# wejpurvis/DIS_project

Hardware: AMD Instinct MI355X
Metric: log-marginal-likelihood evals/sec + fp64 Cholesky GFLOP/s at N=16384 (higher is better)
Workload: dtype f64; 1 GPU; configs[1]: one MLL eval per rank, 64 genes x 256 timepoints, N=16384, fp64; N=16384, genes=64, parallelism=replicas1, exchange=none

## Files before the change

### dis_project_amd/csrc/lfm_chol.hip

```cpp
#include <cstdint>

#include "lfm_chol.h"
#include "lfm_chol_dev.h"

namespace lfm {

static constexpr int STEP_KS = 16;
constexpr int PANEL_TIMEOUT = STATUS_TIMEOUT;
__device__ __forceinline__ void timeout_at(int* status, int why) {
  atomicMin(status, PANEL_TIMEOUT);
  atomicCAS(status + 1, 0, why);
}

template <int SRC>
__device__ __forceinline__ double row_bcast_t(double v) {
  const long long b = __double_as_longlong(v);
  const int lo = __builtin_amdgcn_mov_dpp((int)b, 0x150 + SRC, 0xf, 0xf, false);
  const int hi = __builtin_amdgcn_mov_dpp((int)(b >> 32), 0x150 + SRC, 0xf, 0xf, false);
  return __longlong_as_double(((long long)hi << 32) | (unsigned)lo);
}
__device__ __forceinline__ double row_bcast(double v, int src) {
  switch (src) {
    case 0: return row_bcast_t<0>(v);
    case 1: return row_bcast_t<1>(v);
    case 2: return row_bcast_t<2>(v);
    case 3: return row_bcast_t<3>(v);
    case 4: return row_bcast_t<4>(v);
    case 5: return row_bcast_t<5>(v);
    case 6: return row_bcast_t<6>(v);
    case 7: return row_bcast_t<7>(v);
    case 8: return row_bcast_t<8>(v);
    case 9: return row_bcast_t<9>(v);
    case 10: return row_bcast_t<10>(v);
    case 11: return row_bcast_t<11>(v);
    case 12: return row_bcast_t<12>(v);
    case 13: return row_bcast_t<13>(v);
    case 14: return row_bcast_t<14>(v);
    default: return row_bcast_t<15>(v);
  }
}

template <int SRC>
__device__ __forceinline__ double row_bcast64_t(double v) {
  return __builtin_amdgcn_mov_dpp(v, 0x150 + SRC, 0xf, 0xf, false);
}
__device__ __forceinline__ double row_bcast64(double v, int src) {
  switch (src) {
    case 0: return row_bcast64_t<0>(v);
    case 1: return row_bcast64_t<1>(v);
    case 2: return row_bcast64_t<2>(v);
    case 3: return row_bcast64_t<3>(v);
    case 4: return row_bcast64_t<4>(v);
    case 5: return row_bcast64_t<5>(v);
    case 6: return row_bcast64_t<6>(v);
    case 7: return row_bcast64_t<7>(v);
    case 8: return row_bcast64_t<8>(v);
    case 9: return row_bcast64_t<9>(v);
    case 10: return row_bcast64_t<10>(v);
    case 11: return row_bcast64_t<11>(v);
    case 12: return row_bcast64_t<12>(v);
    case 13: return row_bcast64_t<13>(v);
    case 14: return row_bcast64_t<14>(v);
    default: return row_bcast64_t<15>(v);
  }
}

__device__ __forceinline__ void pin16(double (&p)[16]) {
  asm volatile("" : "+v"(p[0]), "+v"(p[1]), "+v"(p[2]), "+v"(p[3]), "+v"(p[4]), "+v"(p[5]),
               "+v"(p[6]), "+v"(p[7]), "+v"(p[8]), "+v"(p[9]), "+v"(p[10]), "+v"(p[11]),
               "+v"(p[12]), "+v"(p[13]), "+v"(p[14]), "+v"(p[15]));
}

template <bool COH>
__device__ __forceinline__ void st1(double* p, double v) {
  if (COH) __hip_atomic_store(p, v, __ATOMIC_RELAXED, __HIP_MEMORY_SCOPE_AGENT);
  else *p = v;
}
typedef unsigned u32x4v __attribute__((ext_vector_type(4)));
__device__ __forceinline__ void st2_wt(double* base, unsigned off, double a, double b) {
  const __amdgpu_buffer_rsrc_t r = __builtin_amdgcn_make_buffer_rsrc(base, 0, 0x7fffffff, 0x00020000);
  const double2v v = {a, b};
  __builtin_amdgcn_raw_buffer_store_b128(__builtin_bit_cast(u32x4v, v), r, off, 0, 16 );
}
template <bool COH>
__device__ __forceinline__ double ld1(const double* p) {
  if (COH) return __hip_atomic_load(p, __ATOMIC_RELAXED, __HIP_MEMORY_SCOPE_AGENT);
  return *p;
}

__device__ __forceinline__ double rsqrt_nr(double x) {
  double y = __builtin_amdgcn_rsq(x);
  y = y * fma(-0.5 * x * y, y, 1.5);
  y = y * fma(-0.5 * x * y, y, 1.5);
  return y;
}


template <int PH>
__device__ __forceinline__ void potrf_block(double* __restrict__ Mb, double* __restrict__ A,
                                            int64_t lda, int64_t kb, int64_t npiv,
                                            double* __restrict__ dinv,
                                            double* __restrict__ parts, int k,
                                            int* __restrict__ status,
                                            double* __restrict__ Li = nullptr,
                                            unsigned long long* __restrict__ pst = nullptr) {
  auto pstamp = [&](int p) {
    if (pst && threadIdx.x == 0) pst[p] = __builtin_amdgcn_s_memrealtime();
  };
  __shared__ double pvs[NB];
  __shared__ double ipv[NB];
  __shared__ double red[4];
  __shared__ int redi[4];
  int tid = threadIdx.x;
  asm volatile("" : "+v"(tid));
  const int lane = tid & 63, w = tid >> 6;
  const int li = lane & 15, lk = lane >> 4;
#define MS(r, q) Mb[((((r) >> 4) * (((r) >> 4) + 1) / 2) + ((q) >> 4)) * (IB * (IB + 1)) + \
                    ((r) & 15) * (IB + 1) + ((q) & 15)]

  constexpr int LB = (PH & 32) ? 32 : 16;
#pragma unroll
  for (int hb = 0; hb < 32 / LB; ++hb) {
    double2 v[LB];
#pragma unroll
    for (int u = 0; u < LB; ++u) {
      const int idx = tid + 256 * (u + LB * hb), r = idx >> 6, c2 = idx & 63;
      if ((2 * c2) >> 4 <= r >> 4)
        v[u] = (PH & 8) ? ld2<(PH & 16) != 0>(&A[(kb + r) * lda + kb + 2 * c2])
                        : double2{(r == 2 * c2) ? 2.0 : 0.0, (r == 2 * c2 + 1) ? 2.0 : 0.0};
    }
#pragma unroll
    for (int u = 0; u < LB; ++u) {
      const int idx = tid + 256 * (u + LB * hb), r = idx >> 6, c2 = idx & 63;
      if ((2 * c2) >> 4 <= r >> 4) {
        MS(r, 2 * c2) = v[u].x;
        MS(r, 2 * c2 + 1) = v[u].y;
      }
    }
  }
  __syncthreads();

  auto leaf = [&](int cb) {
    const int c0 = cb * IB;
    double d[IB], pv[IB], yv[IB];
#pragma unroll
    for (int q = 0; q < IB; ++q) d[q] = (lane < IB && q <= lane) ? MS(c0 + li, c0 + q) : 0.0;
    if constexpr ((PH & 128) != 0) {
      double dc = row_bcast64(d[0], 0);
      if (kb + c0 >= npiv) dc = 1.0;
      double y = rsqrt_1nr(dc);
#pragma unroll
      for (int c = 0; c < IB; ++c) {
        pv[c] = dc;
        yv[c] = y;
        d[c] = (lane == c) ? dc * y : d[c] * y;
        if (c + 1 < IB) {
          d[c + 1] = fma(-d[c], row_bcast64(d[c], c + 1), d[c + 1]);
          double dn = row_bcast64(d[c + 1], c + 1);
          if (kb + c0 + c + 1 >= npiv) dn = 1.0;
          const double r = __builtin_amdgcn_rsq(dn);
          const double hh = -0.5 * dn;
          const int REM = IB - c - 2, K = (REM + 3) / 4;
          double t1 = 0.0, t2 = 0.0, yn = 0.0;
#pragma unroll
          for (int part = 0; part < 4; ++part) {
            double bq[4];
#pragma unroll
            for (int i = 0; i < 4; ++i) {
              const int q = c + 2 + part * K + i;
              if (i < K && q < IB) bq[i] = row_bcast64(d[c], q);
            }
            __builtin_amdgcn_sched_barrier(0);
#pragma unroll
            for (int i = 0; i < 4; ++i) {
              const int q = c + 2 + part * K + i;
              if (i < K && q < IB) d[q] = fma(-d[c], bq[i], d[q]);
            }
            if (part == 0) t1 = hh * r;
            if (part == 1) t2 = fma(t1, r, 1.5);
            if (part == 2) yn = r * t2;
            __builtin_amdgcn_sched_barrier(0);
          }
          dc = dn;
          y = yn;
        }
      }
    } else {
#pragma unroll
      for (int c = 0; c < IB; ++c) {
        double dc = row_bcast(d[c], c);
        if (kb + c0 + c >= npiv) dc = 1.0;
        const double y = rsqrt_1nr(dc);
        pv[c] = dc;
        yv[c] = y;
        d[c] = (lane == c) ? dc * y : d[c] * y;
#pragma unroll
        for (int q = c + 1; q < IB; ++q) d[q] = fma(-d[c], row_bcast(d[c], q), d[q]);
      }
    }
    if (lane < IB) {
#pragma unroll
      for (int q = 0; q < IB; ++q)
        if (q <= lane) MS(c0 + lane, c0 + q) = d[q];
    }
    double pvl = 0.0, yvl = 0.0;
#pragma unroll
    for (int c = 0; c < IB; ++c) {
      pvl = (lane == c) ? pv[c] : pvl;
      yvl = (lane == c) ? yv[c] : yvl;
    }
    if (lane < IB) {
      pvs[c0 + lane] = pvl;
      ipv[c0 + lane] = yvl;
    }
  };
  auto tile_update = [&](int i0, int j0, int c0) {
    const int bi = __builtin_amdgcn_readfirstlane(i0 >> 4);
    const int bj = __builtin_amdgcn_readfirstlane(j0 >> 4);
    const int bc = __builtin_amdgcn_readfirstlane(c0 >> 4);
    double* C = Mb + (bi * (bi + 1) / 2 + bj) * (IB * (IB + 1));
    const double* Pa = Mb + (bi * (bi + 1) / 2 + bc) * (IB * (IB + 1));
    const double* Pb = Mb + (bj * (bj + 1) / 2 + bc) * (IB * (IB + 1));
    double4v acc;
#pragma unroll
    for (int r = 0; r < 4; ++r) acc[r] = C[(lk + 4 * r) * (IB + 1) + li];
#pragma unroll
    for (int ks = 0; ks < IB / 4; ++ks)
      acc = mfma16(-Pa[li * (IB + 1) + ks * 4 + lk], Pb[li * (IB + 1) + ks * 4 + lk], acc);
#pragma unroll
    for (int r = 0; r < 4; ++r) C[(lk + 4 * r) * (IB + 1) + li] = acc[r];
  };
  auto tri_tile = [](int t, int* ti, int* tj) {
    int r = 0;
    while ((r + 1) * (r + 2) / 2 <= t) ++r;
    *ti = r;
    *tj = t - r * (r + 1) / 2;
  };
#define LI(r, q) Li[((((r) >> 4) * (((r) >> 4) + 1) / 2) + ((q) >> 4)) * (IB * (IB + 1)) + \
                    ((r) & 15) * (IB + 1) + ((q) & 15)]
  auto sweep_pinned = [](double (&p)[IB], const double* Ld, const double* y) {
    double lc[IB], ln[IB], yc = y[0], yn = 0.0;
#pragma unroll
    for (int q = 1; q < IB; ++q) lc[q] = Ld[q * (IB + 1)];
#pragma unroll
    for (int c = 0; c < IB; ++c) {
      if (c + 1 < IB) {
        yn = y[c + 1];
#pragma unroll
        for (int q = c + 2; q < IB; ++q) ln[q] = Ld[q * (IB + 1) + c + 1];
      }
      p[c] = p[c] * yc;
#pragma unroll
      for (int q = c + 1; q < IB; ++q) p[q] = fma(-p[c], lc[q], p[q]);
      pin16(p);
      yc = yn;
#pragma unroll
      for (int q = c + 2; q < IB; ++q) lc[q] = ln[q];
    }
  };
  auto dinv_block = [&](int I) {
    const int c0 = I * IB;
    const int bd = __builtin_amdgcn_readfirstlane(I);
    const double* Ld = Mb + (bd * (bd + 1) / 2 + bd) * (IB * (IB + 1));
    double x[IB];
#pragma unroll
    for (int r = 0; r < IB; ++r) x[r] = (li == r) ? 1.0 : 0.0;
    if constexpr ((PH & 512) != 0) {
      sweep_pinned(x, Ld, ipv + c0);
    } else {
#pragma unroll
      for (int r = 0; r < IB; ++r) {
        x[r] = x[r] * ipv[c0 + r];
#pragma unroll
        for (int q = r + 1; q < IB; ++q) x[q] = fma(-Ld[q * (IB + 1) + r], x[r], x[q]);
      }
    }
    if (lane < IB) {
#pragma unroll
      for (int r = 0; r < IB; ++r) LI(c0 + r, c0 + lane) = x[r];
    }
  };
  auto linv_block = [&](int I, int J) {
    I = __builtin_amdgcn_readfirstlane(I);
    J = __builtin_amdgcn_readfirstlane(J);
    auto blk = [&](int bi, int bj) { return (bi * (bi + 1) / 2 + bj) * (IB * (IB + 1)); };
    double4v sacc = {0, 0, 0, 0};
    for (int K = J; K < I; ++K) {
      const double* a = Mb + blk(I, K);
      const double* b = Li + blk(K, J);
#pragma unroll
      for (int ks = 0; ks < IB / 4; ++ks)
        sacc = mfma16(a[li * (IB + 1) + 4 * ks + lk], b[(4 * ks + lk) * (IB + 1) + li], sacc);
    }
    const double* d = Li + blk(I, I);
    double4v o = {0, 0, 0, 0};
#pragma unroll
    for (int ks = 0; ks < IB / 4; ++ks) o = mfma16(d[li * (IB + 1) + 4 * ks + lk], sacc[ks], o);
    double* out = Li + blk(I, J);
#pragma unroll
    for (int r = 0; r < 4; ++r) out[(lk + 4 * r) * (IB + 1) + li] = -o[r];
  };
  if ((PH & 1) && w == 0) leaf(0);
  __syncthreads();
  pstamp(0);
#pragma unroll 1
  for (int ib = 0; ib < NB / IB; ++ib) {
// ... 624 lines not shown
  double* Xb = g.X + (i0 - g.tr0 + wr + lk) * W + c0 + wc + li;
#pragma unroll
  for (int ir = 0; ir < 8; ++ir)
#pragma unroll
    for (int jr = 0; jr < JR; ++jr) {
      Xb[(ir * 4) * W + jr * 16] = ACC(ir, jr);
      if (i0 + wr + ir * 4 + lk == g.n) g.zvec[g.tk0 + c0 + wc + jr * 16 + li] = ACC(ir, jr);
    }
#undef ACC
  if (st) {
    __syncthreads();
    stamp_max(st + 3);
    add_dur(6);
  }
  return true;
}

template <int TR>
__device__ __forceinline__ void step_body(const StepArgs& g, unsigned long long* ran = nullptr) {
  constexpr int SUB = ST / TR;
  __shared__ double sPbuf[(64 + ST) * (STEP_KS + LDP)];
  double (*sP)[KB + LDP] = reinterpret_cast<double (*)[KB + LDP]>(sPbuf);
  double (*sPu)[STEP_KS + LDP] = reinterpret_cast<double (*)[STEP_KS + LDP]>(sPbuf);
  const int64_t b = blockIdx.x;
  const int cnt[3] = {g.na, g.nr, g.nt};
  const int64_t width[2] = {pad8(g.na), pad8(g.nr)};
  int seg = 0;
  int64_t base = 0;
  while (seg < 2 && b >= base + width[seg]) {
    base += width[seg];
    ++seg;
  }
  int64_t lo, hi;
  tall_or_xcd_range(seg, cnt[seg], b - base, &lo, &hi);
  const int64_t u = lo;
  if (u >= hi) return;
  const int role = seg + 1;
  if (ran && threadIdx.x == 0) *ran = ((unsigned long long)role << 32) | (unsigned long long)u;
  unsigned long long* const st = g.stamps;
  if (st) stamp_max(st, true);
  const unsigned long long t_unit = st ? __builtin_amdgcn_s_memrealtime() : 0;
  auto add_dur = [&](int slot) {
    if (threadIdx.x == 0)
      __hip_atomic_fetch_add(st + slot, __builtin_amdgcn_s_memrealtime() - t_unit,
                             __ATOMIC_RELAXED, __HIP_MEMORY_SCOPE_AGENT);
  };
  if (role == 1) {
    syrk_unit<true, TR, true, STEP_KS>(g.A, g.lda, g.s0, g.px, g.kd, g.T, 0, g.wn, u, g.wn, sPu,
                                       0, g.n, g.pad_end, g.zero_from,
                                       g.gen.tab ? &g.gen : nullptr);
    __builtin_amdgcn_s_waitcnt(0);
    __syncthreads();
    const int trow = g.wn + (int)(u / (SUB * g.wn));
    if (threadIdx.x == 0 && g.a_done)
      __hip_atomic_fetch_add(&g.a_done[trow], 1u, __ATOMIC_RELAXED, __HIP_MEMORY_SCOPE_AGENT);
    if (threadIdx.x == 0 && g.xready && trow < g.wn + g.lead)
      __hip_atomic_fetch_add(g.xready, 1u, __ATOMIC_RELAXED, __HIP_MEMORY_SCOPE_AGENT);
    if (st) {
      stamp_max(st + 1);
      stamp_max(st + 3);
      add_dur(7);
    }
    return;
  }
  if (role == 2) {
    unsigned long long c0 = 0, r0 = 0;
    if (st) {
      c0 = __builtin_amdgcn_s_memtime();
      r0 = __builtin_amdgcn_s_memrealtime();
    }
    const bool lead = syrk_unit<true, TR, false, STEP_KS>(g.A, g.lda, g.s0, g.px, g.kd, g.T,
                                                          g.wn, g.T, u + g.rest_off, 0, sPu,
                                                          g.xready ? g.wn + g.lead : 0, g.n,
                                                          g.pad_end, g.zero_from,
                                                          g.gen.tab ? &g.gen : nullptr);
    if (lead) bump_after_stores(g.xready);
    if (st) {
      __syncthreads();
      stamp_max(st + 1);
      stamp_max(st + 3);
      if (threadIdx.x == 0) {
        __hip_atomic_fetch_add(st + 4, __builtin_amdgcn_s_memtime() - c0, __ATOMIC_RELAXED,
                               __HIP_MEMORY_SCOPE_AGENT);
        __hip_atomic_fetch_add(st + 5, __builtin_amdgcn_s_memrealtime() - r0, __ATOMIC_RELAXED,
                               __HIP_MEMORY_SCOPE_AGENT);
      }
    }
    return;
  }
  tall_unit(g, u, sP, st, t_unit);
}

template <int TR>
__device__ __forceinline__ void step_traced(const StepArgs& g) {
  __shared__ unsigned long long t0;
  __shared__ unsigned long long ran;
  if (threadIdx.x == 0) {
    t0 = __builtin_amdgcn_s_memrealtime();
    ran = 0;
  }
  __syncthreads();
  step_body<TR>(g, &ran);
  __syncthreads();
  if (threadIdx.x == 0) {
    const int64_t b = blockIdx.x;
    unsigned hw, xcc;
    asm volatile("s_getreg_b32 %0, hwreg(HW_REG_HW_ID)" : "=s"(hw));
    asm volatile("s_getreg_b32 %0, hwreg(HW_REG_XCC_ID)" : "=s"(xcc));
    unsigned long long* r = g.trace + 4 * b;
    r[0] = t0;
    r[1] = __builtin_amdgcn_s_memrealtime();
    r[2] = (unsigned long long)hw | ((unsigned long long)xcc << 32);
    r[3] = (g.trace_tag << 40) | ran;
  }
}

__global__ __launch_bounds__(256, 4) void step_kernel(StepArgs g) { step_body<64>(g); }
__global__ __launch_bounds__(256, 4) void helper_update_kernel(StepArgs g) { step_body<64>(g); }
__global__ __launch_bounds__(256, 4) void step_kernel_traced(StepArgs g) { step_traced<64>(g); }
__global__ __launch_bounds__(256, 4) void helper_update_kernel_traced(StepArgs g) {
  step_traced<64>(g);
}

static_assert(MB_DOUBLES >= 64 * (NB + 1) && MB_DOUBLES >= (64 + ST) * (KB + LDP), "LDS union");

__device__ __forceinline__ bool wait_counter(unsigned* p, unsigned target, unsigned limit,
                                             const int* status) {
  __shared__ int ok;
  if (threadIdx.x == 0) ok = spin_until<true>(p, target, limit, status);
  __syncthreads();
  __builtin_amdgcn_fence(__ATOMIC_ACQUIRE, "agent");
  return ok;
}

__global__ __launch_bounds__(256) void panel_kernel(double* __restrict__ A, int64_t lda,
                                                    int64_t kb, int64_t pkb, int pkd,
                                                    int64_t npiv, double* __restrict__ dinv,
                                                    double* __restrict__ parts, int k,
                                                    int* __restrict__ status,
                                                    unsigned* __restrict__ sync, unsigned epoch,
                                                    unsigned spin) {
  extern __shared__ __attribute__((aligned(16))) double smem[];
  __builtin_amdgcn_s_setprio(3);
  const int tid = threadIdx.x, lane = tid & 63, w = tid >> 6;
  const int wr = (w >> 1) * 32, wc = (w & 1) * 64;
  const int li = lane & 15, lk = lane >> 4;
  const int b = blockIdx.x;
  const int64_t i0 = b < 2 ? kb + 64 * b : kb + NB + 64 * (int64_t)(b - 2);
  double* Cb = A + (i0 + wr + lk) * lda + kb + wc + li;
  const int ld4 = (int)(4 * lda);
  double acc[8][4];
#pragma unroll
  for (int ir = 0; ir < 8; ++ir)
#pragma unroll
    for (int jr = 0; jr < 4; ++jr) acc[ir][jr] = -Cb[ir * ld4 + jr * 16];
  if (pkd > 0)
    gemm_accumulate<64>(A + i0 * lda + pkb, lda, A + kb * lda + pkb, lda, pkd, acc,
                        reinterpret_cast<double (*)[KB + LDP]>(smem));
  if (b < 2) {
#pragma unroll
    for (int ir = 0; ir < 8; ++ir)
#pragma unroll
      for (int jr = 0; jr < 4; ++jr) Cb[ir * ld4 + jr * 16] = -acc[ir][jr];
    __threadfence();
    __syncthreads();
    if (tid == 0) __hip_atomic_fetch_add(&sync[1], 1u, __ATOMIC_RELEASE, __HIP_MEMORY_SCOPE_AGENT);
    if (b == 1) return;
    if (!wait_counter(&sync[1], 2u * epoch, spin, status)) {
      if (tid == 0) {
        timeout_at(status, 7);
        __hip_atomic_store(&sync[0], epoch, __ATOMIC_RELEASE, __HIP_MEMORY_SCOPE_AGENT);
      }
      return;
    }
    potrf_block<15>(smem, A, lda, kb, npiv, dinv, parts, k, status);
    __threadfence();
    __syncthreads();
    if (tid == 0) __hip_atomic_store(&sync[0], epoch, __ATOMIC_RELEASE, __HIP_MEMORY_SCOPE_AGENT);
    return;
  }
  double (*sA)[NB + 1] = reinterpret_cast<double (*)[NB + 1]>(smem);
  __syncthreads();
#pragma unroll
  for (int ir = 0; ir < 8; ++ir)
#pragma unroll
    for (int jr = 0; jr < 4; ++jr) sA[wr + ir * 4 + lk][wc + jr * 16 + li] = -acc[ir][jr];
  if (!wait_counter(&sync[0], epoch, spin, status)) {
    if (tid == 0) timeout_at(status, 7);
    return;
  }
  trsm_rows(sA, A, lda, i0, kb, dinv);
}


__device__ __forceinline__ bool grid_sync(unsigned* bar, unsigned target, int* status,
                                          unsigned limit) {
  __shared__ int ok;
  __syncthreads();
  if (threadIdx.x == 0) {
    __threadfence();
    __hip_atomic_fetch_add(bar, 1u, __ATOMIC_RELEASE, __HIP_MEMORY_SCOPE_AGENT);
    const bool good = spin_until<true, 1>(bar, target, limit, status);
    if (!good) timeout_at(status, 6);
    ok = good;
  }
  __syncthreads();
  __builtin_amdgcn_fence(__ATOMIC_ACQUIRE, "agent");
  return ok;
}

__device__ __forceinline__ bool grid_sync_light(unsigned* bar, unsigned target, int* status,
                                                unsigned limit) {
  __shared__ int ok;
  __builtin_amdgcn_s_waitcnt(0);
  __syncthreads();
  if (threadIdx.x == 0) {
    __hip_atomic_fetch_add(bar, 1u, __ATOMIC_RELAXED, __HIP_MEMORY_SCOPE_AGENT);
    const bool good = spin_until<false, 1>(bar, target, limit, status);
    if (!good) timeout_at(status, 6);
    ok = good;
  }
  __syncthreads();
  return ok;
}


constexpr int CKS = 64;
static_assert(2 * MB_DOUBLES >= (64 + ST) * (CKS + LDP), "chain LDS union");

constexpr int G32K = 129;
static_assert(2 * MB_DOUBLES >= 2 * 32 * G32K + 4 * 1024 && 2 * MB_DOUBLES >= 4 * 32 * 33,
              "gemm32 LDS (+ the in-chain solve's parked output tiles)");
template <bool BT, bool COH = false, bool PAIR = false>
__device__ __forceinline__ void gemm32(const double* __restrict__ pi, int64_t ldi,
                                       const double* __restrict__ pj, int64_t ldj, int kd,
                                       double (&v)[4], double* __restrict__ smem) {
  int tid = threadIdx.x;
  asm volatile("" : "+v"(tid));
  const int lane = tid & 63, w = tid >> 6;
  const int li = lane & 15, lk = lane >> 4;
  double* sA = smem;
  double* sB = smem + 32 * G32K;
  double4v acc4[2][2];
#pragma unroll
  for (int rb = 0; rb < 2; ++rb) acc4[rb][0] = acc4[rb][1] = (double4v){0.0, 0.0, 0.0, 0.0};
#define ACC(ir, jr) acc4[(ir) >> 2][jr][(ir) & 3]
  double2 pre[16];
  auto gload = [&](int k0) {
#pragma unroll
    for (int u = 0; u < 8; ++u) {
      const int idx = tid + 256 * u;
      pre[u] = ld2<COH>(pi + (idx >> 6) * ldi + k0 + 2 * (idx & 63));
      pre[8 + u] = BT ? ld2<COH>(pj + (int64_t)(k0 + (idx >> 4)) * ldj + 2 * (idx & 15))
                      : ld2<COH>(pj + (idx >> 6) * ldj + k0 + 2 * (idx & 63));
    }
  };
  if (kd > 0) gload(0);
  for (int k0 = 0; k0 < kd; k0 += 128) {
    __syncthreads();
#pragma unroll
    for (int u = 0; u < 8; ++u) {
      const int idx = tid + 256 * u;
      double* d = sA + (idx >> 6) * G32K + 2 * (idx & 63);
      d[0] = pre[u].x;
      d[1] = pre[u].y;
      if (BT) {
        const int kr = idx >> 4, c = 2 * (idx & 15);
        sB[c * G32K + kr] = pre[8 + u].x;
        sB[(c + 1) * G32K + kr] = pre[8 + u].y;
      } else {
        double* e = sB + (idx >> 6) * G32K + 2 * (idx & 63);
        e[0] = pre[8 + u].x;
        e[1] = pre[8 + u].y;
      }
    }
    __syncthreads();
    if (k0 + 128 < kd) gload(k0 + 128);
#pragma unroll
    for (int kk = 32 * w; kk < 32 * w + 32; kk += 4) {
      const double b0 = sB[li * G32K + kk + lk], b1 = sB[(16 + li) * G32K + kk + lk];
      const double a0 = sA[li * G32K + kk + lk], a1 = sA[(16 + li) * G32K + kk + lk];
      acc4[0][0] = mfma16(a0, b0, acc4[0][0]);
      acc4[0][1] = mfma16(a0, b1, acc4[0][1]);
      acc4[1][0] = mfma16(a1, b0, acc4[1][0]);
      acc4[1][1] = mfma16(a1, b1, acc4[1][1]);
    }
  }
  __syncthreads();
  double* red = smem;
#pragma unroll
  for (int ir = 0; ir < 8; ++ir)
#pragma unroll
    for (int jr = 0; jr < 2; ++jr) red[(w * 32 + ir * 4 + lk) * 33 + jr * 16 + li] = ACC(ir, jr);
#undef ACC
  __syncthreads();
#pragma unroll
  for (int q = 0; q < 4; ++q) {
    const int e = PAIR ? 2 * tid + 512 * (q >> 1) + (q & 1) : tid + 256 * q, r = e >> 5, c = e & 31;
    v[q] = red[r * 33 + c] + red[(32 + r) * 33 + c] + red[(64 + r) * 33 + c] +
           red[(96 + r) * 33 + c];
  }
  __syncthreads();
}
template <bool LIGHT>
__global__ __launch_bounds__(256) void chain_kernel(ChainArgs g) {
  extern __shared__ __attribute__((aligned(16))) double smem[];
  const int G = gridDim.x, wg = blockIdx.x, tid = threadIdx.x;
  const int W = g.w * NB;
  double* Aw = g.Wk - (g.Kc * W + g.Kc);
  unsigned nbar = 0;
  auto stamp = [&](int p) {
    if (g.stamps && wg == 0 && tid == 0 && p < 16) g.stamps[p] = __builtin_amdgcn_s_memrealtime();
  };
  auto sync = [&]() {
    return (LIGHT ? grid_sync_light : grid_sync)(g.bar, G * ++nbar, g.status, g.spin >> 2);
  };
  stamp(0);
  if (g.xready) {
    __shared__ int okx;
    if (tid == 0) {
      okx = spin_until<false>(g.xready, g.xtarget, g.spin, g.status);
      if (!okx) timeout_at(g.status, 5);
    }
    __syncthreads();
    if (!LIGHT) __builtin_amdgcn_fence(__ATOMIC_ACQUIRE, "agent");
    if (!okx) return;
  }
  stamp(14);
  if (g.kd > 0) {
    const int nc = g.kd / 32, nu = (W / 32) * nc;
    for (int u = wg; u < nu; u += G) {
      const int cb = u % nc, rb = u / nc;
      const int kd = min(g.kd, (32 * (cb + 1) + 127) / 128 * 128);
      double v[4];
      gemm32<true, LIGHT, LIGHT>(g.A + (g.Kc + 32 * rb) * g.lda + g.K0p, g.lda, g.Bdp + 32 * cb,
                                 g.kd, kd, v, smem);
      if (LIGHT) {
#pragma unroll
        for (int h = 0; h < 2; ++h) {
          const int e = 2 * tid + 512 * h;
          st2_wt(g.xd, (unsigned)(((32 * rb + (e >> 5)) * g.kd + 32 * cb + (e & 31)) * 8), v[2 * h],
                 v[2 * h + 1]);
        }
      } else {
#pragma unroll
        for (int q = 0; q < 4; ++q) {
          const int e = tid + 256 * q;
          g.xd[(int64_t)(32 * rb + (e >> 5)) * g.kd + 32 * cb + (e & 31)] = v[q];
        }
      }
    }
    if (!sync()) return;
  }
  stamp(13);
  {
    const int nt = W / 32, ntile = nt * (nt + 1) / 2;
    for (int u = wg; u < ntile; u += G) {
      int ti = 0;
      while ((ti + 1) * (ti + 2) / 2 <= u) ++ti;
      const int tj = u - ti * (ti + 1) / 2;
      double v[4] = {0.0, 0.0, 0.0, 0.0};
      if (g.kd > 0)
        gemm32<false, LIGHT, LIGHT>(g.xd + (int64_t)32 * ti * g.kd, g.kd,
                                    g.xd + (int64_t)32 * tj * g.kd, g.kd, g.kd, v, smem);
      if (LIGHT) {
#pragma unroll
        for (int h = 0; h < 2; ++h) {
          const int e = 2 * tid + 512 * h;
          const int il = 32 * ti + (e >> 5), jl = 32 * tj + (e & 31);
          const double2 a = ld2<true>(&g.A[(g.Kc + il) * g.lda + g.Kc + jl]);
          st2_wt(g.Wk, (unsigned)((il * W + jl) * 8), a.x - v[2 * h], a.y - v[2 * h + 1]);
        }
      } else {
#pragma unroll
        for (int q = 0; q < 4; ++q) {
          const int e = tid + 256 * q;
          const int64_t i = g.Kc + 32 * ti + (e >> 5), j = g.Kc + 32 * tj + (e & 31);
          Aw[i * W + j] = g.A[i * g.lda + j] - v[q];
        }
      }
    }
    for (int64_t idx = (int64_t)wg * 256 + tid; idx < (LIGHT ? 0 : (int64_t)W * W / 2);
         idx += (int64_t)G * 256) {
      const int r = (int)(idx / (W / 2)), c = 2 * (int)(idx % (W / 2));
      double2 v;
      v.x = (r == c) ? 1.0 : 0.0;
      v.y = (r == c + 1) ? 1.0 : 0.0;
      *reinterpret_cast<double2*>(&g.Wk[(int64_t)(W + r) * W + c]) = v;
    }
  }
  stamp(1);
  bool ok = sync();
  stamp(2);
  for (int c = 0; c < g.w && ok; ++c) {
    const int64_t kb = g.Kc + (int64_t)c * NB, r0 = kb + NB;
    if (wg == 0) {
      double* Li = smem + MB_DOUBLES;
      potrf_block<(LIGHT ? 127 : 47) | 128 | 512>(smem, Aw, W, kb, g.n, g.dinv, g.parts,
                                                  (int)(kb / NB), g.status, Li,
                                                  g.stamps && g.w == 1 ? g.stamps + 5 : nullptr);
      stamp(3 + 3 * c);
      store_inverse_t<LIGHT>(Li, g.w == 1 ? g.Wk + (int64_t)W * W : g.linv, g.w == 1 ? W : NB);
      stamp(4 + 3 * c);
    }
    if (g.w == 1) break;
    ok = sync();
    if (!ok) break;
    const int64_t rows = g.Kc + 2 * W - r0;
    {
      double* park = smem + 2 * 32 * G32K;
      for (int64_t u = wg; u < rows / 32; u += G) {
        const int64_t ra = r0 + 32 * u;
#pragma unroll 1
        for (int jc = 0; jc < 4; ++jc) {
          double v[4];
          gemm32<true>(Aw + ra * W + kb, W, g.linv + 32 * jc, NB, NB, v, smem);
#pragma unroll
          for (int q = 0; q < 4; ++q) park[jc * 1024 + tid + 256 * q] = v[q];
        }
        __syncthreads();
#pragma unroll
        for (int jc = 0; jc < 4; ++jc)
#pragma unroll
          for (int q = 0; q < 4; ++q) {
            const int e = tid + 256 * q;
            Aw[(ra + (e >> 5)) * W + kb + 32 * jc + (e & 31)] = park[jc * 1024 + e];
          }
        __syncthreads();
      }
    }
    ok = sync();
    stamp(5 + 3 * c);
    if (!ok || c + 1 == g.w) break;
    const int hi = g.w - 1 - c;
    {
      const int R32 = (int)(rows / 32), J32 = 4 * hi;
      int nt = 0;
      for (int jt = 0; jt < J32; ++jt) nt += R32 - jt;
      for (int u = wg; u < nt; u += G) {
        int jt = 0, rem = u;
        while (rem >= R32 - jt) {
          rem -= R32 - jt;
          ++jt;
        }
        const int it = jt + rem;
        const int64_t ra = r0 + 32 * it, ca = r0 + 32 * jt;
        double v[4];
        gemm32<false>(Aw + ra * W + kb, W, Aw + ca * W + kb, W, NB, v, smem);
#pragma unroll
        for (int q = 0; q < 4; ++q) {
          const int e = tid + 256 * q;
          Aw[(ra + (e >> 5)) * W + ca + (e & 31)] -= v[q];
        }
      }
    }
    ok = sync();
  }
  if (wg == 0) {
    if (g.n >= g.Kc && g.n < g.Kc + W) {
      const int r = (int)(g.n - g.Kc);
      for (int c = tid; c < W; c += 256)
        g.zvec[g.Kc + c] = !LIGHT ? g.Wk[(int64_t)r * W + c]
                           : c <= r ? smem[(((r >> 4) * ((r >> 4) + 1) / 2) + (c >> 4)) *
                                               (IB * (IB + 1)) + (r & 15) * (IB + 1) + (c & 15)]
                                    : 0.0;
    }
    if (LIGHT) __builtin_amdgcn_s_waitcnt(0);
    else __threadfence();
    __syncthreads();
    stamp(15);
    if (tid == 0)
      __hip_atomic_store(g.done, 1u, LIGHT ? __ATOMIC_RELAXED : __ATOMIC_RELEASE,
                         __HIP_MEMORY_SCOPE_AGENT);
  }
}

__global__ __launch_bounds__(256) void coresident_kernel(unsigned* bar, int* ok) {
  extern __shared__ double pad[];
  if (threadIdx.x == 0) {
    pad[0] = 0.0;
    __hip_atomic_fetch_add(bar, 1u, __ATOMIC_RELAXED, __HIP_MEMORY_SCOPE_AGENT);
    unsigned it = 0;
    while (__hip_atomic_load(bar, __ATOMIC_RELAXED, __HIP_MEMORY_SCOPE_AGENT) < gridDim.x &&
           ++it < (1u << 20))
      __builtin_amdgcn_s_sleep(2);
    if (it >= (1u << 20)) atomicExch(ok, 0);
  }
}

__global__ __launch_bounds__(1024) void finalize_kernel(const double* __restrict__ A, int64_t lda,
                                                        int64_t n, const double* __restrict__ parts,
                                                        int nparts, const int* __restrict__ status,
                                                        int negative, double* __restrict__ out,
                                                        const double* __restrict__ zvec,
                                                        int64_t zsplit) {
  __shared__ double red[2][16];
  const int tid = threadIdx.x;
  double q = 0.0, ld = 0.0;
  for (int64_t c = tid; c < n; c += 1024) {
    const double z = c < zsplit ? zvec[c] : A[n * lda + c];
    q += z * z;
  }
  for (int k = tid; k < nparts; k += 1024) ld += parts[k];
  for (int o = 32; o > 0; o >>= 1) {
    q += __shfl_xor(q, o);
    ld += __shfl_xor(ld, o);
  }
  if ((tid & 63) == 0) {
    red[0][tid >> 6] = q;
    red[1][tid >> 6] = ld;
  }
  __syncthreads();
  if (tid == 0) {
    double Q = 0.0, LD = 0.0;
    for (int i = 0; i < 16; ++i) {
      Q += red[0][i];
      LD += red[1][i];
    }
    const double logdet = 2.0 * LD;
    const double two_pi = 6.283185307179586476925;
    double mll = -0.5 * ((double)n * log(two_pi) + logdet + Q);
    mll *= negative ? -1.0 : 1.0;
    if (status[0] != STATUS_NONE) mll = __builtin_nan("");
    out[0] = mll;
    out[1] = logdet;
    out[2] = Q;
    out[3] = (double)status[0];
    out[4] = (double)status[1];
  }
}

__global__ void status_init_kernel(int* st) {
  st[0] = STATUS_NONE;
  st[1] = 0;
}

const void* chol_kernel_template(int i) {
  static const void* const k[6] = {reinterpret_cast<const void*>(&potrf_diag_kernel<15>),
                                   reinterpret_cast<const void*>(&syrk_kernel<true, 64>),
                                   reinterpret_cast<const void*>(&syrk_kernel<true, 128>),
                                   reinterpret_cast<const void*>(&syrk_kernel<false, 64>),
                                   reinterpret_cast<const void*>(&chain_kernel<false>),
                                   reinterpret_cast<const void*>(&chain_kernel<true>)};
  return k[i];
}

}
```

### dis_project_amd/csrc/lfm_host.h

```cpp
#pragma once

#include <atomic>
#include <cmath>
#include <cstdint>
#include <mutex>
#include <shared_mutex>
#include <string>
#include <tuple>
#include <utility>
#include <vector>

#include "lfm_mid_plan.h"
#include "lfm_small_plan.h"

namespace lfm {

LFM_HD inline int gene_index(double g, int G) {
  double tg = trunc(g);
  if (tg < 0) tg += (double)G;
  if (!(tg >= 0)) tg = 0;
  if (tg > (double)(G - 1)) tg = (double)(G - 1);
  return (int)tg;
}
LFM_HD inline long long flag_int(double f) {
  double tf = trunc(f);
  if (!(tf == tf)) return 0;
  if (tf > 4e18) tf = 4e18;
  if (tf < -4e18) tf = -4e18;
  return (long long)tf;
}

struct GridLayout {
  bool ok = false;
  int T = 0;
  int nblk = 0;
  double t0 = 0, dt = 0;
  std::vector<double> times;
  std::vector<int> block_gene;
};

GridLayout detect_grid(const double* x, int64_t n, int64_t G);
inline int small_grid_T(const GridLayout& lay, int64_t G) {
  return lay.ok && tables_doubles((int)G, lay.T) <= (size_t)SMALL_GRID_TAB_MAX ? lay.T : 0;
}

std::vector<std::pair<int64_t, int>> plan_steps(int64_t nblk, int64_t Mp, int nb, bool bordered,
                                                bool s3, int wbulk, int64_t w4min,
                                                int64_t w2min, int w0 = 1);

constexpr int kBandMaxCols = 8;

void rest_unit_tile(int64_t b, int T, int tj_lo, int Q, int* ti_out, int* tj_out);

int64_t helper_units(int kd, int na, int nr, int nt, int wnext, int nb, int cus, int side_cus,
                     double tc, double dmin);

int64_t helper_clamp(int64_t hu, int nr, int T, int wn, int lead, int Q);

LFM_HD constexpr int64_t pad8(int units) { return (int64_t)(units + 7) / 8 * 8; }
LFM_HD constexpr int64_t tall_grid(int64_t nt, int split) {
  return (nt + 8 * split - 1) / (8 * split) * (8 * split);
}

constexpr size_t chol_events(int S) { return 3 * (size_t)S + 3; }

struct S3Params {
  int64_t n = 0, Mp = 0;
  bool bordered = false, fused = false, prof = false;
  int nb = 128, st = 128, tall_split = 2, supertile = 6;
  int cus = 256, side_cus = 32;
  int helper = 1;
  double helper_tc = 700, helper_min = 1200;
  int64_t ovl_at = 6144;
};
inline bool operator==(const S3Params& a, const S3Params& b) {
  auto t = [](const S3Params& p) {
    return std::tie(p.n, p.Mp, p.bordered, p.fused, p.prof, p.nb, p.st, p.tall_split, p.supertile,
                    p.cus, p.side_cus, p.helper, p.helper_tc, p.helper_min, p.ovl_at);
  };
  return t(a) == t(b);
}

struct S3Step {
  int64_t K0 = 0, K1 = 0;
  int w = 0, kd = 0;
  int T = 0, wn = 0;
  int na = 0, nr = 0;
  int nt = 0, tw = 0;
  int64_t tr0 = 0, tk0 = 0;
  int64_t zero_from = INT64_MAX, copy_from = INT64_MAX;
  bool gen = false;
  int lead = 0;
  unsigned xtarget = 0;
  int64_t hu = 0;
  int nr_main = 0;
  size_t f_done = 0, f_adone = 0, f_bar = 0, f_xready = 0;
  int64_t grid = 0;
  int64_t hgrid = 0;
  int64_t ugrid = 0, tgrid = 0;
  bool ovl_mark = false;
  size_t wk_off = 0, bd_off = 0, x_off = 0;
  double step_alg = 0, step_issued = 0, upd_alg = 0, upd_issued = 0, tall_alg = 0,
         tall_issued = 0, helper_alg = 0, helper_issued = 0, chain_alg = 0, chain_issued = 0;
};

struct S3Plan {
  S3Params params;
  std::vector<std::pair<int64_t, int>> step_list;
  int S = 0;
  int64_t Wmax = 0, Tmax = 0;
  size_t wk_bytes = 0, xbuf_bytes = 0, zvec_bytes = 0, linv_bytes = 0, xd_bytes = 0,
         flags_bytes = 0;
  size_t nflags = 0, chain_done = 0, a_done = 0, bars = 0, xready = 0;
  int64_t pad_end = 0, zsplit = 0;
  size_t nevents = 0;
  std::vector<S3Step> steps;
};

S3Plan plan_s3(const std::vector<std::pair<int64_t, int>>& steps, const S3Params& p);
bool plan_s3_keep(S3Plan& kept, const std::vector<std::pair<int64_t, int>>& steps,
                  const S3Params& p);

constexpr int POST_W = 4;
constexpr size_t POST_VT_BUDGET = (size_t)1 << 30;
constexpr int64_t POST_CHUNK_MAX = 16384;

struct PostChunk {
  int64_t q0 = 0, rows = 0;
  int64_t pad_rows = 0;
  int panel_grid = 0;
  int tiles = 0;
};
struct PostPanel {
  int64_t K0 = 0, K1 = 0;
  int w = 0;
  int tj0 = 0, ntj = 0;
};
struct ResidentPlan {
  enum Reject { OK = 0, BAD_M, COV_CHUNK, BAD_CHUNK };
  int reject = OK;
  std::string why;
  int64_t n = 0, Np = 0, m = 0, chunk = 0;
  std::vector<PostChunk> chunks;
  std::vector<PostPanel> panels;
  int64_t vt_rows = 0;
  size_t vt_bytes = 0;
  size_t acc_bytes = 0;
  size_t t_bytes = 0;
  size_t out_bytes = 0;
  size_t cov_bytes = 0;
  int cov_tiles = 0;
};
int64_t post_default_chunk(int64_t Np);
ResidentPlan plan_post(int64_t n, int64_t G, int64_t m, int64_t chunk, bool want_cov);

LFM_HD inline void philox4x32_10(uint32_t c[4], uint32_t k0, uint32_t k1) {
  constexpr uint32_t M0 = 0xD2511F53u, M1 = 0xCD9E8D57u, W0 = 0x9E3779B9u, W1 = 0xBB67AE85u;
  for (int r = 0; r < 10; ++r) {
    const uint64_t p0 = (uint64_t)M0 * c[0], p1 = (uint64_t)M1 * c[2];
    const uint32_t n0 = (uint32_t)(p1 >> 32) ^ c[1] ^ k0, n2 = (uint32_t)(p0 >> 32) ^ c[3] ^ k1;
    c[0] = n0;
    c[1] = (uint32_t)p1;
    c[2] = n2;
    c[3] = (uint32_t)p0;
    k0 += W0;
    k1 += W1;
  }
}
LFM_HD inline void sample_uniforms(uint64_t seed, uint64_t s, uint64_t p, double* u1, double* u2) {
  uint32_t c[4] = {(uint32_t)p, (uint32_t)(p >> 32), (uint32_t)s, (uint32_t)(s >> 32)};
  philox4x32_10(c, (uint32_t)seed, (uint32_t)(seed >> 32));
  const uint64_t a = ((uint64_t)c[0] | (uint64_t)c[1] << 32) >> 11;
  const uint64_t b = ((uint64_t)c[2] | (uint64_t)c[3] << 32) >> 11;
  *u1 = (double)(a + 1) * 0x1p-53;
  *u2 = (double)(b + 1) * 0x1p-53;
}

constexpr int64_t SAMPLE_MAX_NSAMP = (int64_t)1 << 24;
constexpr int64_t SAMPLE_RANDN_GRID = 1 << 16;
struct SamplePlan {
  enum Reject { OK = 0, BAD_N, BAD_NSAMP, BAD_SAMPLE0, RANGE, TOO_MANY };
  int reject = OK;
  std::string why;
  int64_t n = 0, nsamp = 0, sample0 = 0;
  int64_t Np = 0, Mp = 0;
  int64_t ldz = 0, zrows = 0;
  size_t mat_bytes = 0;
  size_t z_bytes = 0;
  size_t x_bytes = 0;
  int tiles_i = 0, tiles_j = 0;
  int64_t pairs = 0;
  int randn_grid = 0;
};
inline int sample_tile_col(const SamplePlan& P, int by) { return P.tiles_j - 1 - by; }
inline int64_t sample_depth(int tj) { return 128 * ((int64_t)tj + 1); }
SamplePlan plan_sample(int64_t n, int64_t nsamp, int64_t sample0);

class TenancyLock {
 public:
  bool open(const std::string& path);
  void lock_exclusive();
  void unlock_exclusive();
  void lock_shared();
  void unlock_shared();
  std::string path();
  int error() const { return err_.load(std::memory_order_acquire); }
  ~TenancyLock();

 private:
  bool files() const;
  void fail(int e, const char* what);
  std::atomic<int> err_{0};
  bool fd_held_ = false;
  bool sh_held_ = false;
  std::shared_mutex rw_;
  std::mutex turn_mu_;
  std::mutex fd_mu_;
  std::mutex open_mu_;
  int readers_ = 0;
  int fd_ = -1, turn_ = -1;
  bool opened_ = false, ok_ = false;
  std::string path_;
};

}
```

Baseline: 36.39 MLL evals/s.

## Add 64x64 MFMA GEMM tiles and trim chain solve/update to live rows

Adds a gemm64 routine that computes 64x64 fp64 tiles with MFMA, using four waves each owning a 32x32 quadrant with register prefetch. The chain kernel's projection, SYRK and trailing band-update phases now use it when there are enough tiles to fill the grid, with the 32x32 path kept as fallback. Separately, the triangular solve and band update now cover only rows that are live for the current window instead of the full 2W extent, which removes redundant work. The larger tiles raise register and LDS pressure and reduce the number of parallel units available in small phases.

```diff
diff --git a/dis_project_amd/csrc/lfm_chol.hip b/dis_project_amd/csrc/lfm_chol.hip
--- a/dis_project_amd/csrc/lfm_chol.hip
+++ b/dis_project_amd/csrc/lfm_chol.hip
@@ -2,6 +2,7 @@
 
 #include "lfm_chol.h"
 #include "lfm_chol_dev.h"
+#include "lfm_host.h"
 
 namespace lfm {
 
@@ -1232,6 +1233,94 @@
   }
   __syncthreads();
 }
+
+constexpr int G64K = 64 + LDP;
+static_assert(2 * MB_DOUBLES >= 2 * 64 * G64K, "gemm64 LDS");
+template <bool BT>
+__device__ __forceinline__ void gemm64(const double* __restrict__ pi, int64_t ldi,
+                                       const double* __restrict__ pj, int64_t ldj, int kd,
+                                       double (&v)[16], double* __restrict__ smem) {
+  int tid = threadIdx.x;
+  asm volatile("" : "+v"(tid));
+  const int lane = tid & 63, w = tid >> 6;
+  const int li = lane & 15, lk = lane >> 4;
+  const int wr = (w >> 1) * 32, wc = (w & 1) * 32;
+  double* sA = smem;
+  double* sB = smem + 64 * G64K;
+  double4v acc[4][2][2];
+#pragma unroll
+  for (int q = 0; q < 4; ++q)
+#pragma unroll
+    for (int rb = 0; rb < 2; ++rb)
+      acc[q][rb][0] = acc[q][rb][1] = (double4v){0.0, 0.0, 0.0, 0.0};
+  double2 pre[16];
+  auto gload = [&](int k0) {
+#pragma unroll
+    for (int u = 0; u < 8; ++u) {
+      const int idx = tid + 256 * u;
+      pre[u] = ld2<false>(pi + (idx >> 5) * ldi + k0 + 2 * (idx & 31));
+      pre[8 + u] = BT ? ld2<false>(pj + (int64_t)(k0 + (idx >> 5)) * ldj + 2 * (idx & 31))
+                      : ld2<false>(pj + (idx >> 5) * ldj + k0 + 2 * (idx & 31));
+    }
+  };
+  if (kd > 0) gload(0);
+  for (int k0 = 0; k0 < kd; k0 += 128) {
+#pragma unroll
+    for (int h = 0; h < 2; ++h) {
+      __syncthreads();
+#pragma unroll
+      for (int u = 0; u < 8; ++u) {
+        const int idx = tid + 256 * u;
+        double* d = sA + (idx >> 5) * G64K + 2 * (idx & 31);
+        d[0] = pre[u].x;
+        d[1] = pre[u].y;
+        if (BT) {
+          const int kr = idx >> 5, c = 2 * (idx & 31);
+          sB[c * G64K + kr] = pre[8 + u].x;
+          sB[(c + 1) * G64K + kr] = pre[8 + u].y;
+        } else {
+          double* e = sB + (idx >> 5) * G64K + 2 * (idx & 31);
+          e[0] = pre[8 + u].x;
+          e[1] = pre[8 + u].y;
+        }
+      }
+      __syncthreads();
+      if (k0 + 64 * h + 64 < kd) gload(k0 + 64 * h + 64);
+#pragma unroll
+      for (int q2 = 0; q2 < 2; ++q2)
+#pragma unroll
+        for (int kk = 32 * q2; kk < 32 * q2 + 32; kk += 4) {
+          const int q = 2 * h + q2;
+          const double b0 = sB[(wc + li) * G64K + kk + lk], b1 = sB[(wc + 16 + li) * G64K + kk + lk];
+          const double a0 = sA[(wr + li) * G64K + kk + lk], a1 = sA[(wr + 16 + li) * G64K + kk + lk];
+          acc[q][0][0] = mfma16(a0, b0, acc[q][0][0]);
+          acc[q][0][1] = mfma16(a0, b1, acc[q][0][1]);
+          acc[q][1][0] = mfma16(a1, b0, acc[q][1][0]);
+          acc[q][1][1] = mfma16(a1, b1, acc[q][1][1]);
+        }
+    }
+  }
+#pragma unroll
+  for (int rb = 0; rb < 2; ++rb)
+#pragma unroll
+    for (int jr = 0; jr < 2; ++jr)
+#pragma unroll
+      for (int r = 0; r < 4; ++r)
+        v[4 * (2 * rb + jr) + r] =
+            acc[0][rb][jr][r] + acc[1][rb][jr][r] + acc[2][rb][jr][r] + acc[3][rb][jr][r];
+}
+template <class F>
+__device__ __forceinline__ void gemm64_each(const double (&v)[16], bool skip_upper, F f) {
+  const int lane = threadIdx.x & 63, w = threadIdx.x >> 6;
+  if (skip_upper && w == 1) return;
+  const int r0 = (w >> 1) * 32 + (lane >> 4), c0 = (w & 1) * 32 + (lane & 15);
+#pragma unroll
+  for (int rb = 0; rb < 2; ++rb)
+#pragma unroll
+    for (int jr = 0; jr < 2; ++jr)
+#pragma unroll
+      for (int r = 0; r < 4; ++r) f(r0 + 16 * rb + 4 * r, c0 + 16 * jr, v[4 * (2 * rb + jr) + r]);
+}
 template <bool LIGHT>
 __global__ __launch_bounds__(256) void chain_kernel(ChainArgs g) {
   extern __shared__ __attribute__((aligned(16))) double smem[];
@@ -1259,7 +1348,17 @@
   stamp(14);
   if (g.kd > 0) {
     const int nc = g.kd / 32, nu = (W / 32) * nc;
-    for (int u = wg; u < nu; u += G) {
+    const bool wide = !LIGHT && nu / 4 >= G;
+    if constexpr (!LIGHT) for (int u = wg; wide && u < nu / 4; u += G) {
+      const int cb = u % (nc / 2), rb = u / (nc / 2);
+      const int kd = min(g.kd, (64 * (cb + 1) + 127) / 128 * 128);
+      double v[16];
+      gemm64<true>(g.A + (g.Kc + 64 * rb) * g.lda + g.K0p, g.lda, g.Bdp + 64 * cb, g.kd, kd, v,
+                   smem);
+      double* xt = g.xd + (int64_t)64 * rb * g.kd + 64 * cb;
+      gemm64_each(v, false, [&](int r, int c, double x) { xt[(int64_t)r * g.kd + c] = x; });
+    }
+    for (int u = wg; !wide && u < nu; u += G) {
       const int cb = u % nc, rb = u / nc;
       const int kd = min(g.kd, (32 * (cb + 1) + 127) / 128 * 128);
       double v[4];
@@ -1285,7 +1384,24 @@
   stamp(13);
   {
     const int nt = W / 32, ntile = nt * (nt + 1) / 2;
-    for (int u = wg; u < ntile; u += G) {
+    const int nt64 = W / 64, ntile64 = nt64 * (nt64 + 1) / 2;
+    const bool wide = !LIGHT && ntile64 >= G;
+    if constexpr (!LIGHT) for (int u = wg; wide && u < ntile64; u += G) {
+      int ti = 0;
+      while ((ti + 1) * (ti + 2) / 2 <= u) ++ti;
+      const int tj = u - ti * (ti + 1) / 2;
+      double v[16];
+#pragma unroll
+      for (int q = 0; q < 16; ++q) v[q] = 0.0;
+      if (g.kd > 0)
+        gemm64<false>(g.xd + (int64_t)64 * ti * g.kd, g.kd, g.xd + (int64_t)64 * tj * g.kd, g.kd,
+                      g.kd, v, smem);
+      const int64_t i0 = g.Kc + 64 * ti, j0 = g.Kc + 64 * tj;
+      gemm64_each(v, ti == tj, [&](int r, int c, double x) {
+        Aw[(i0 + r) * W + j0 + c] = g.A[(i0 + r) * g.lda + j0 + c] - x;
+      });
+    }
+    for (int u = wg; !wide && u < ntile; u += G) {
       int ti = 0;
       while ((ti + 1) * (ti + 2) / 2 <= u) ++ti;
       const int tj = u - ti * (ti + 1) / 2;
@@ -1336,11 +1452,11 @@
     if (g.w == 1) break;
     ok = sync();
     if (!ok) break;
-    const int64_t rows = g.Kc + 2 * W - r0;
     {
       double* park = smem + 2 * 32 * G32K;
-      for (int64_t u = wg; u < rows / 32; u += G) {
-        const int64_t ra = r0 + 32 * u;
+      const int nsolve = chain_solve_units(g.w, c, 32, true);
+      for (int u = wg; u < nsolve; u += G) {
+        const int64_t ra = r0 + 32 * chain_solve_unit(g.w, c, 32, u);
 #pragma unroll 1
         for (int jc = 0; jc < 4; ++jc) {
           double v[4];
@@ -1362,18 +1478,21 @@
     ok = sync();
     stamp(5 + 3 * c);
     if (!ok || c + 1 == g.w) break;
-    const int hi = g.w - 1 - c;
     {
-      const int R32 = (int)(rows / 32), J32 = 4 * hi;
-      int nt = 0;
-      for (int jt = 0; jt < J32; ++jt) nt += R32 - jt;
-      for (int u = wg; u < nt; u += G) {
-        int jt = 0, rem = u;
-        while (rem >= R32 - jt) {
-          rem -= R32 - jt;
-          ++jt;
-        }
-        const int it = jt + rem;
+      const int nt64 = chain_band_tiles(g.w, c, 64, true);
+      const bool wide = !LIGHT && nt64 >= G;
+      if constexpr (!LIGHT) for (int u = wg; wide && u < nt64; u += G) {
+        int it, jt;
+        chain_band_tile(g.w, c, 64, true, u, &it, &jt);
+        const int64_t ra = r0 + 64 * it, ca = r0 + 64 * jt;
+        double v[16];
+        gemm64<false>(Aw + ra * W + kb, W, Aw + ca * W + kb, W, NB, v, smem);
+        gemm64_each(v, it == jt, [&](int r, int cc, double x) { Aw[(ra + r) * W + ca + cc] -= x; });
+      }
+      const int nt = chain_band_tiles(g.w, c, 32, true);
+      for (int u = wg; !wide && u < nt; u += G) {
+        int it, jt;
+        chain_band_tile(g.w, c, 32, true, u, &it, &jt);
         const int64_t ra = r0 + 32 * it, ca = r0 + 32 * jt;
         double v[4];
         gemm32<false>(Aw + ra * W + kb, W, Aw + ca * W + kb, W, NB, v, smem);
diff --git a/dis_project_amd/csrc/lfm_host.h b/dis_project_amd/csrc/lfm_host.h
--- a/dis_project_amd/csrc/lfm_host.h
+++ b/dis_project_amd/csrc/lfm_host.h
@@ -60,6 +60,37 @@
 LFM_HD constexpr int64_t pad8(int units) { return (int64_t)(units + 7) / 8 * 8; }
 LFM_HD constexpr int64_t tall_grid(int64_t nt, int split) {
   return (nt + 8 * split - 1) / (8 * split) * (8 * split);
+}
+
+LFM_HD constexpr int chain_units_per_block(int t) { return 128 / t; }
+LFM_HD constexpr int chain_rows_full(int w, int c, int t) {
+  return chain_units_per_block(t) * (2 * w - 1 - c);
+}
+LFM_HD constexpr int chain_rows_live(int w, int , int t) {
+  return chain_units_per_block(t) * w;
+}
+LFM_HD constexpr bool chain_row_is_live(int w, int c, int t, int ru) {
+  const int d = chain_units_per_block(t) * (w - 1 - c);
+  return ru < d || (ru - d) / chain_units_per_block(t) <= c;
+}
+LFM_HD constexpr int chain_solve_units(int w, int c, int t, bool live) {
+  return live ? chain_rows_live(w, c, t) : chain_rows_full(w, c, t);
+}
+LFM_HD constexpr int chain_solve_unit(int , int , int , int u) { return u; }
+LFM_HD constexpr int chain_band_tiles(int w, int c, int t, bool live) {
+  const int R = live ? chain_rows_live(w, c, t) : chain_rows_full(w, c, t);
+  const int J = chain_units_per_block(t) * (w - 1 - c);
+  return J * R - J * (J - 1) / 2;
+}
+LFM_HD inline void chain_band_tile(int w, int c, int t, bool live, int u, int* it, int* jt) {
+  const int R = live ? chain_rows_live(w, c, t) : chain_rows_full(w, c, t);
+  int j = 0, rem = u;
+  while (rem >= R - j) {
+    rem -= R - j;
+    ++j;
+  }
+  *it = j + rem;
+  *jt = j;
 }
 
 constexpr size_t chol_events(int S) { return 3 * (size_t)S + 3; }
```

New measurement: 36.61 MLL evals/s (median of 6 runs). About the same (+0.6%).
